# BraveGroup/DCD

Measured on AMD Instinct MI355X. Metric: images/sec DGDE train step (bs=8, 384x1280), higher is better.
Workload: dtype f32; 1 GPU; DGDE train bs=8 fp32 on 1xMI355X, synthetic KITTI 384x1280 + random kpts_ann (DGDE.yaml, DLA-34+DCNv2, 6 objects/image); global_batch=8, per_gpu_batch=8, input=384x1280, parallelism=dp1, dcn_precision=f32, step_launch=eager, sync_bn=False

## Files before the change

### dcd_amd/csrc/conv.hip

```cpp
#include <hip/hip_runtime.h>
#include <stdint.h>
#include <stdlib.h>

#include "../../include/dcd_hip.h"
#include "tuning_env.h"
#include "lds_limit.h"
#include "bf16_split.h"

typedef float f32x16 __attribute__((ext_vector_type(16)));
typedef float f32x4 __attribute__((ext_vector_type(4)));
typedef float f32x2 __attribute__((ext_vector_type(2)));

namespace {

constexpr int WN_CH = 8;
constexpr int WN_NT = 512;

template <int TR, int TC, int NB>
struct WinoGeom {
    static constexpr int KS = 32 * NB;
    static constexpr int U = 16 * KS * WN_CH;
    static constexpr int NTILE = TR * TC;
    static constexpr int ROWS = 4 * TR + 2;
    static constexpr int Q = (2 * TC + 8) / 4;
    static constexpr int RS = TC == 16 ? 48 : 42;
    static constexpr int PLANE = ROWS * RS;
    static constexpr int IN = WN_CH * PLANE;
    static constexpr int BUF = IN + U;
    static_assert(NTILE <= 32 && 4 * Q <= RS && RS % 2 == 0 && (2 * TC) % 4 == 0, "region geometry");
};

__device__ __forceinline__ void win_read4(const float *e, float (&q)[4])
{
    const f32x2 a = *reinterpret_cast<const f32x2 *>(e), b = *reinterpret_cast<const f32x2 *>(e + 2),
                c = *reinterpret_cast<const f32x2 *>(e + 4);
    q[0] = a.y; q[1] = b.x; q[2] = b.y; q[3] = c.x;
}

template <int RS>
__device__ __forceinline__ void win_store4(float *d, const f32x4 v)
{
    if constexpr (RS % 4 == 0) {
        *reinterpret_cast<f32x4 *>(d) = v;
    } else {
        *reinterpret_cast<f32x2 *>(d) = f32x2{v.x, v.y};
        *reinterpret_cast<f32x2 *>(d + 2) = f32x2{v.z, v.w};
    }
}

__device__ __forceinline__ void xcd_remap(int &bx, int &by)
{
    const int gx = gridDim.x, NT = gx * gridDim.y;
    const int L = bx + gx * by;
    const int xc = L & 7, slot = L >> 3;
    const int q = NT >> 3, r = NT & 7;
    const int Lp = (xc < r ? xc * (q + 1) : r * (q + 1) + (xc - r) * q) + slot;
    by = Lp / gx;
    bx = Lp - by * gx;
}

__device__ __forceinline__ void wino_prep_body(const float *__restrict__ w, float *__restrict__ ul, int Cc, int Kk, int mode, int nchunk,
                                               int nz, int WN_KS, int first, int step)
{
    const int n = nz * nchunk * WN_KS * WN_CH;
    for (int idx = first; idx < n; idx += step) {
        int r = idx;
        const int s = r & 3; r >>= 2;
        const int h = r & 1; r >>= 1;
        const int kk = r % WN_KS; r /= WN_KS;
        const int ck = r % nchunk, z = r / nchunk;
        const int k = z * WN_KS + kk, c = ck * WN_CH + 2 * s + h;
        float g[3][3];
#pragma unroll
        for (int a = 0; a < 3; ++a)
#pragma unroll
            for (int b = 0; b < 3; ++b) {
                float v = 0.f;
                if (k < Kk && c < Cc)
                    v = mode == 0 ? w[(((size_t)k * Cc + c) * 3 + a) * 3 + b] : w[(((size_t)c * Kk + k) * 3 + (2 - a)) * 3 + (2 - b)];
                g[a][b] = v;
            }
        float t[4][3];
#pragma unroll
        for (int b = 0; b < 3; ++b) {
            t[0][b] = g[0][b];
            t[1][b] = 0.5f * (g[0][b] + g[1][b] + g[2][b]);
            t[2][b] = 0.5f * (g[0][b] - g[1][b] + g[2][b]);
            t[3][b] = g[2][b];
        }
#pragma unroll
        for (int xi = 0; xi < 4; ++xi) {
            const float u[4] = {t[xi][0], 0.5f * (t[xi][0] + t[xi][1] + t[xi][2]), 0.5f * (t[xi][0] - t[xi][1] + t[xi][2]), t[xi][2]};
#pragma unroll
            for (int nu = 0; nu < 4; ++nu)
                ul[((((size_t)(z * nchunk + ck) * 16 + xi * 4 + nu) * 2 + h) * WN_KS + kk) * 4 + s] = u[nu];
        }
    }
}

__global__ void wino_prep_weights(const float *__restrict__ w, float *__restrict__ ul, int Cc, int Kk, int mode, int nchunk, int nz,
                                  int WN_KS)
{
    wino_prep_body(w, ul, Cc, Kk, mode, nchunk, nz, WN_KS, blockIdx.x * blockDim.x + threadIdx.x, gridDim.x * blockDim.x);
}

struct PrepBoth {
    float *ul[2];
    int Cc[2], Kk[2], nchunk[2], nz[2], ks[2];
};

__global__ void wino_prep_weights_both(const float *__restrict__ w, PrepBoth p)
{
    const int mode = blockIdx.y;
    if (!p.ul[mode]) return;
    wino_prep_body(w, p.ul[mode], p.Cc[mode], p.Kk[mode], mode, p.nchunk[mode], p.nz[mode], p.ks[mode],
                   blockIdx.x * blockDim.x + threadIdx.x, gridDim.x * blockDim.x);
}

__global__ void wino_prep_weights_table(const long long *__restrict__ table)
{
    const long long *e = table + 5 * (size_t)blockIdx.z;
    const float *w = reinterpret_cast<const float *>(e[0]);
    const int mode = blockIdx.y;
    float *ul = reinterpret_cast<float *>(e[1 + mode]);
    if (!w || !ul) return;
    const int Cin = (int)e[3], Cout = (int)e[4];
    const int Cc = mode ? Cout : Cin, Kk = mode ? Cin : Cout;
    const int WN_KS = Kk <= 32 ? 32 : 64;
    wino_prep_body(w, ul, Cc, Kk, mode, (Cc + WN_CH - 1) / WN_CH, (Kk + WN_KS - 1) / WN_KS, WN_KS,
                   blockIdx.x * blockDim.x + threadIdx.x, gridDim.x * blockDim.x);
}

template <int TR, int TC, int NB>
__global__ __launch_bounds__(WN_NT) void wino_conv3x3_f32(const float *__restrict__ x, const float *__restrict__ ul, float *y,
                                                          float *__restrict__ part, const float *__restrict__ bias,
                                                          const float *residual, int Cc, int H, int W, int Kk, int tiles_x,
                                                          int nchunk, int nz)
{
    using G = WinoGeom<TR, TC, NB>;
    constexpr int WN_ROWS = G::ROWS, WN_RS = G::RS, WN_PLANE = G::PLANE, WN_IN = G::IN, WN_BUF = G::BUF, WN_Q = G::Q;
    constexpr int WN_KS = G::KS, WN_U = G::U;
    extern __shared__ __attribute__((aligned(16))) float lds[];
    const int tid = threadIdx.x;
    const int lane = tid & 63, wave = tid >> 6;
    const int p = lane & 31, h = lane >> 5;
    const int xi = wave & 3, tg = wave >> 2;
    int bx = blockIdx.x, b = blockIdx.y;
    xcd_remap(bx, b);
    const int ty = bx / tiles_x, tx = bx - ty * tiles_x;
    const int r0 = ty * (4 * TR), c0 = tx * (2 * TC);
    const int z = blockIdx.z % nz, ks = blockIdx.z / nz, ksplit = gridDim.z / nz;
    const int ck0 = (int)((int64_t)ks * nchunk / ksplit), ck1 = (int)((int64_t)(ks + 1) * nchunk / ksplit);
    const int HW = H * W;
    const bool live = p < G::NTILE;
    const int pe = live ? p : 0;
    const int trow = pe / TC, tcol = pe - trow * TC;

    const int ra = xi == 0 ? 0 : 1, rb = xi == 3 ? 3 : 2;
    const float sa = xi == 2 ? -1.f : 1.f, sb = (xi == 0 || xi == 3) ? -1.f : 1.f;
    const int lanebase = (2 * TR * tg + 2 * trow) * WN_RS + 2 + 2 * tcol + h * WN_PLANE;
    const int base1 = lanebase + ra * WN_RS, base2 = lanebase + rb * WN_RS;

    const float *x_b = x + (size_t)b * Cc * HW;
    const float *ul_z = ul + (size_t)z * nchunk * WN_U;

    constexpr int KIN = (WN_CH * WN_ROWS * WN_Q + WN_NT - 1) / WN_NT;
    constexpr int KW = WN_U / 4 / WN_NT;
    int sg[KIN], sl[KIN];
    bool sv_[KIN];
#pragma unroll
    for (int k = 0; k < KIN; ++k) {
        const int e = tid + WN_NT * k;
        const int ch = e / (WN_ROWS * WN_Q), rem = e - ch * (WN_ROWS * WN_Q);
        const int row = rem / WN_Q, q = rem - row * WN_Q;
        const int yy = r0 - 1 + row, xx = c0 - 4 + 4 * q;
        sv_[k] = e < WN_CH * WN_ROWS * WN_Q;
        sg[k] = (sv_[k] && yy >= 0 && yy < H && xx >= 0 && xx < W) ? ch * HW + yy * W + xx : -1;
        sl[k] = ch * WN_PLANE + row * WN_RS + 4 * q;
    }
    f32x4 rin[KIN];
    auto issue_w = [&](int ck, float *buf) {
        const float *src = ul_z + (size_t)ck * WN_U + 4 * tid;
        float *dst = buf + WN_IN + 4 * 64 * __builtin_amdgcn_readfirstlane(wave);
#pragma unroll
        for (int k = 0; k < KW; ++k)
            __builtin_amdgcn_global_load_lds(src + 4 * WN_NT * k, (__attribute__((address_space(3))) void *)(dst + 4 * WN_NT * k), 16, 0, 0);
    };
    auto issue = [&](int ck) {
        const float *src = x_b + (size_t)ck * WN_CH * HW;
        const int cleft = Cc - ck * WN_CH;
#pragma unroll
        for (int k = 0; k < KIN; ++k) {
            const f32x4 zero4 = {0.f, 0.f, 0.f, 0.f};
            rin[k] = zero4;
            if (sv_[k] && sg[k] >= 0 && (tid + WN_NT * k) / (WN_ROWS * WN_Q) < cleft) rin[k] = *reinterpret_cast<const f32x4 *>(src + sg[k]);
        }
    };
    auto commit = [&](float *buf) {
#pragma unroll
        for (int k = 0; k < KIN; ++k)
            if (sv_[k]) win_store4<WN_RS>(buf + sl[k], rin[k]);
    };

    f32x16 acc[4][NB];
#pragma unroll
    for (int nu = 0; nu < 4; ++nu)
#pragma unroll
        for (int mb = 0; mb < NB; ++mb)
#pragma unroll
            for (int r = 0; r < 16; ++r) acc[nu][mb][r] = 0.f;

    issue_w(ck0, lds);
    issue(ck0);
    commit(lds);
    asm volatile("s_waitcnt vmcnt(0)" ::: "memory");
    __syncthreads();

    for (int ck = ck0; ck < ck1; ++ck) {
        const float *buf = lds + ((ck - ck0) & 1) * WN_BUF;
#ifndef WN_ABL_NOSTAGE
        if (ck + 1 < ck1) {
            issue_w(ck + 1, lds + ((ck + 1 - ck0) & 1) * WN_BUF);
            issue(ck + 1);
        }
#endif
        const float *ub = buf + WN_IN + ((xi * 4 * 2 + h) * WN_KS + p) * 4;
        const float *cp1 = buf + base1, *cp2 = buf + base2;
        f32x4 a0[4], a1[4];
#pragma unroll
        for (int nu = 0; nu < 4; ++nu) {
            a0[nu] = *reinterpret_cast<const f32x4 *>(ub + (nu * WN_KS) * 8);
            if (NB == 2) a1[nu] = *reinterpret_cast<const f32x4 *>(ub + (nu * WN_KS) * 8 + 32 * 4);
        }
        float qa[4], qb[4];
#ifndef WN_ABL_NOLDS
        win_read4(cp1, qa);
        win_read4(cp2, qb);
#endif
#pragma unroll
        for (int s = 0; s < 4; ++s) {
#ifdef WN_ABL_NOLDS
            const float t0 = sa * (float)s, t1 = sb, t2 = sa + sb, t3 = (float)ck;
#else
            const float t0 = sa * qa[0] + sb * qb[0], t1 = sa * qa[1] + sb * qb[1];
            const float t2 = sa * qa[2] + sb * qb[2], t3 = sa * qa[3] + sb * qb[3];
            if (s + 1 < 4) {
                win_read4(cp1 + 2 * (s + 1) * WN_PLANE, qa);
                win_read4(cp2 + 2 * (s + 1) * WN_PLANE, qb);
            }
#endif
            const float v[4] = {t0 - t2, t1 + t2, t2 - t1, t1 - t3};
            __builtin_amdgcn_sched_barrier(0);
#pragma unroll
            for (int nu = 0; nu < 4; ++nu) {
                acc[nu][0] = __builtin_amdgcn_mfma_f32_32x32x2f32(a0[nu][s], v[nu], acc[nu][0], 0, 0, 0);
                if (NB == 2) acc[nu][NB - 1] = __builtin_amdgcn_mfma_f32_32x32x2f32(a1[nu][s], v[nu], acc[nu][NB - 1], 0, 0, 0);
            }
        }
#ifndef WN_ABL_NOSTAGE
        if (ck + 1 < ck1) commit(lds + ((ck + 1 - ck0) & 1) * WN_BUF);
#endif
        asm volatile("s_waitcnt vmcnt(0)" ::: "memory");
        __syncthreads();
    }
#ifdef WN_ABL_NOEPI
    if (acc[0][0][0] != 123.456f) return;
#endif

    float *ex = lds;
    float *y_b = (ks == 0 ? y : part + (size_t)(ks - 1) * gridDim.y * Kk * HW) + (size_t)b * Kk * HW;
    const float *r_b = (residual && ks == 0) ? residual + (size_t)b * Kk * HW : nullptr;
    const int orow0 = r0 + 2 * TR * tg + 2 * trow, ocol = c0 + 2 * tcol;
#pragma unroll
    for (int mb = 0; mb < NB; ++mb) {
        float *mine = ex + (size_t)wave * 32 * 64 + lane;
#pragma unroll
        for (int r = 0; r < 16; ++r) {
            mine[r * 64] = acc[0][mb][r] + acc[1][mb][r] + acc[2][mb][r];
            mine[(16 + r) * 64] = acc[1][mb][r] - acc[2][mb][r] - acc[3][mb][r];
        }
        __syncthreads();
        const float *t0 = ex + (size_t)(tg * 4 + 0) * 32 * 64 + lane, *t1 = t0 + 32 * 64, *t2 = t1 + 32 * 64, *t3 = t2 + 32 * 64;
        if (live && ocol < W) {
#pragma unroll
            for (int rr = 0; rr < 4; ++rr) {
                const int r = 4 * xi + rr;
                const int k = z * WN_KS + mb * 32 + (r & 3) + 8 * (r >> 2) + 4 * h;
                const float a0 = t0[r * 64], a1 = t1[r * 64], a2 = t2[r * 64], a3 = t3[r * 64];
                const float b0 = t0[(16 + r) * 64], b1 = t1[(16 + r) * 64], b2 = t2[(16 + r) * 64], b3 = t3[(16 + r) * 64];
                if (k < Kk) {
                    const float bk = (bias && ks == 0) ? bias[k] : 0.f;
                    const size_t o = (size_t)k * HW + (size_t)orow0 * W + ocol;
                    float *dst = y_b + o;
                    f32x2 r0 = {bk, bk}, r1 = {bk, bk};
                    if (r_b) {
                        if (orow0 < H) r0 += *reinterpret_cast<const f32x2 *>(r_b + o);
                        if (orow0 + 1 < H) r1 += *reinterpret_cast<const f32x2 *>(r_b + o + W);
                    }
                    if (orow0 < H) *reinterpret_cast<f32x2 *>(dst) = f32x2{a0 + a1 + a2 + r0.x, b0 + b1 + b2 + r0.y};
                    if (orow0 + 1 < H) *reinterpret_cast<f32x2 *>(dst + W) = f32x2{a1 - a2 - a3 + r1.x, b1 - b2 - b3 + r1.y};
                }
            }
        }
        __syncthreads();
    }
}

constexpr int WS_CH = 16;

template <int NB>
__device__ __forceinline__ void wino_prep_split_body(const float *__restrict__ w, unsigned *__restrict__ us, int Cc, int Kk, int mode,
                                                     int nchunk, int nz, int first, int step)
{
    constexpr int KS = 32 * NB;
    const int n = nz * nchunk * KS * 2 * 4;
    for (int idx = first; idx < n; idx += step) {
        int r = idx;
        const int d = r & 3; r >>= 2;
        const int h = r & 1; r >>= 1;
        const int kk = r % KS; r /= KS;
        const int ck = r % nchunk, z = r / nchunk;
        const int k = z * KS + kk;
        float u[2][16];
#pragma unroll
        for (int e = 0; e < 2; ++e) {
            const int c = ck * WS_CH + 2 * (2 * d + e) + h;
            float g[3][3];
#pragma unroll
            for (int a = 0; a < 3; ++a)
#pragma unroll
                for (int b = 0; b < 3; ++b) {
                    float v = 0.f;
                    if (k < Kk && c < Cc)
                        v = mode == 0 ? w[(((size_t)k * Cc + c) * 3 + a) * 3 + b] : w[(((size_t)c * Kk + k) * 3 + (2 - a)) * 3 + (2 - b)];
                    g[a][b] = v;
                }
            float t[4][3];
#pragma unroll
            for (int b = 0; b < 3; ++b) {
                t[0][b] = g[0][b];
                t[1][b] = 0.5f * (g[0][b] + g[1][b] + g[2][b]);
                t[2][b] = 0.5f * (g[0][b] - g[1][b] + g[2][b]);
                t[3][b] = g[2][b];
            }
#pragma unroll
            for (int xi = 0; xi < 4; ++xi) {
                u[e][xi * 4 + 0] = t[xi][0];
// ... 500 lines not shown

__global__ __launch_bounds__(256) void wino_wrw_reduce(const float *__restrict__ part, float *__restrict__ gw, int Cin, int Cout, int S,
                                                       int ncg, int KO)
{
    __shared__ float m[12][17];
    const int tid = threadIdx.x;
    const int pos = tid >> 4, l = tid & 15;
    const int gidx = blockIdx.x * 16 + l;
    const int per = KO * 64;
    const int blk = gidx / per, kc = gidx - blk * per;
    if (pos < 12) {
        const float *src = part + ((size_t)blk * S * 12 + pos) * per + kc;
        float sum = 0.f;
#pragma unroll 8
        for (int sp = 0; sp < S; ++sp) sum += src[(size_t)sp * 12 * per];
        m[pos][l] = sum;
    }
    __syncthreads();
    if (pos < 9) {
        const int a = pos / 3, b = pos - a * 3;
        const float ga[4] = {a == 0 ? 1.f : 0.f, 0.5f, a == 1 ? -0.5f : 0.5f, a == 2 ? 1.f : 0.f};
        float r = 0.f;
#pragma unroll
        for (int xi = 0; xi < 4; ++xi) r += ga[xi] * m[xi * 3 + b][l];
        const int og = blk / ncg, cg = blk - og * ncg;
        const int k = og * KO + (kc >> 6), c = cg * 64 + (kc & 63);
        if (k < Cout && c < Cin) gw[((size_t)k * Cin + c) * 9 + pos] = r;
    }
}

}

struct ConvPlan {
    int geom;
    int nb;
    int tiles_x, tiles_y, nchunk, nz, ksplit;
};

static int device_cus()
{
    static int cus = 0;
    if (!cus) {
        int dev = 0, n = 0;
        if (hipGetDevice(&dev) != hipSuccess || hipDeviceGetAttribute(&n, hipDeviceAttributeMultiprocessorCount, dev) != hipSuccess || n <= 0)
            n = 256;
        cus = n;
    }
    return cus;
}

static ConvPlan conv_plan(int B, int Cc, int H, int W, int Kk)
{
    ConvPlan best{};
    const int cus = device_cus();
    int64_t best_cost = -1;
    for (int g = 0; g < 2; ++g) {
        ConvPlan p;
        p.geom = g;
        p.tiles_x = g == 0 ? (W + 31) / 32 : (W + 19) / 20;
        p.tiles_y = g == 0 ? (H + 7) / 8 : (H + 11) / 12;
        p.nchunk = (Cc + WN_CH - 1) / WN_CH;
        p.nb = Kk <= 32 ? 1 : 2;
        p.nz = (Kk + 32 * p.nb - 1) / (32 * p.nb);
        const int64_t wgs = (int64_t)p.tiles_x * p.tiles_y * B * p.nz;
        static const int min_chunks = dcd_env("DCD_CONV_MINCHUNK") ? atoi(dcd_env("DCD_CONV_MINCHUNK")) : 4;
        int ks = 1;
        while (ks < 8 && wgs * (ks * 2) <= cus && p.nchunk / (ks * 2) >= min_chunks) ks *= 2;
        p.ksplit = ks;
        const int64_t rounds = (wgs * ks + cus - 1) / cus;
        const int64_t cost = rounds * ((p.nchunk + ks - 1) / ks + 2) * (g == 0 ? 16 : 17);
        if (best_cost < 0 || cost < best_cost) {
            best_cost = cost;
            best = p;
        }
    }
    return best;
}

template <int TR, int TC, int NB>
static int conv_launch(hipStream_t stream, const ConvPlan &pl, const float *input, const float *ul, float *output, float *part,
                       const float *bias, const float *residual, int B, int Cc, int H, int W, int Kk)
{
    static LdsLimit lds_limit;
    size_t ldsb = (size_t)2 * WinoGeom<TR, TC, NB>::BUF * sizeof(float);
    if (ldsb < (size_t)8 * 32 * 64 * sizeof(float)) ldsb = (size_t)8 * 32 * 64 * sizeof(float);
    if (!lds_limit.raise((int)ldsb, wino_conv3x3_f32<TR, TC, NB>)) return DCD_ERR_LAUNCH;
    hipLaunchKernelGGL((wino_conv3x3_f32<TR, TC, NB>), dim3(pl.tiles_x * pl.tiles_y, B, pl.nz * pl.ksplit), dim3(WN_NT), ldsb, stream,
                       input, ul, output, part, bias, residual, Cc, H, W, Kk, pl.tiles_x, pl.nchunk, pl.nz);
    return DCD_OK;
}

template <int NB, int NP>
static int conv_launch_split(hipStream_t stream, const ConvPlan &pl, const float *input, const unsigned *us, float *output, float *part,
                             const float *bias, const float *residual, int B, int Cc, int H, int W, int Kk)
{
    static LdsLimit lds_limit;
    using G = WinoGeom<2, 16, NB>;
    const size_t ldsb = ((size_t)((WS_CH * G::PLANE + 3) & ~3) + (size_t)2 * 16 * NB * 2 * 256) * sizeof(float);
    if (!lds_limit.raise((int)ldsb, wino_conv3x3_split<NB, NP>)) return DCD_ERR_LAUNCH;
    hipLaunchKernelGGL((wino_conv3x3_split<NB, NP>), dim3(pl.tiles_x * pl.tiles_y, B, pl.nz * pl.ksplit), dim3(WN_NT), ldsb, stream, input,
                       us, output, part, bias, residual, Cc, H, W, Kk, pl.tiles_x, pl.nchunk, pl.nz);
    return DCD_OK;
}

static ConvPlan conv_plan_split(int B, int Cc, int H, int W, int Kk)
{
    ConvPlan p;
    p.geom = 0;
    p.tiles_x = (W + 31) / 32;
    p.tiles_y = (H + 7) / 8;
    p.nchunk = (Cc + WS_CH - 1) / WS_CH;
    p.nb = Kk <= 32 ? 1 : 2;
    p.nz = (Kk + 32 * p.nb - 1) / (32 * p.nb);
    const int64_t wgs = (int64_t)p.tiles_x * p.tiles_y * B * p.nz;
    const int cus = device_cus();
    int ks = 1;
    while (ks < 8 && wgs * (ks * 2) <= cus && p.nchunk / (ks * 2) >= 2) ks *= 2;
    p.ksplit = ks;
    return p;
}

static bool conv_direct_ok(int Cc, int H, int W)
{
    return (int64_t)(Cc + DC_CH) * H * W < (1ll << 29);
}

static ConvPlan conv_plan_direct(int B, int Cc, int H, int W, int Kk)
{
    static const int pin = dcd_env("DCD_CONV_DIRECT_P") ? atoi(dcd_env("DCD_CONV_DIRECT_P")) : 0;
    const int cus = device_cus();
    ConvPlan best{};
    int64_t best_cost = -1;
    for (int P = 2; P <= 4; P += 2) {
        if (P != (pin == 4 ? 4 : 2)) continue;
        ConvPlan p;
        static const int wxpin = dcd_env("DCD_CONV_DIRECT_WX") ? atoi(dcd_env("DCD_CONV_DIRECT_WX")) : 0;
        const int wx = P == 2 && wxpin == 2 ? 2 : 1;
        p.geom = P | (wx << 4);
        p.tiles_x = (W + 32 * wx - 1) / (32 * wx);
        p.tiles_y = (H + 4 * P - 1) / (4 * P);
        p.nchunk = (Cc + DC_CH - 1) / DC_CH;
        p.nb = Kk <= 32 ? 1 : 2;
        p.nz = (Kk + 32 * p.nb - 1) / (32 * p.nb);
        const int64_t wgs = (int64_t)p.tiles_x * p.tiles_y * B * p.nz;
        static const int min_chunks = dcd_env("DCD_CONV_DIRECT_MINCHUNK") ? atoi(dcd_env("DCD_CONV_DIRECT_MINCHUNK")) : 16;
        int ks = 1;
        while (ks < 8) {
            const int64_t next = wgs * ks * 2;
            const int left = p.nchunk / (ks * 2);
            const bool fill = next <= 3 * cus && left >= min_chunks;
            const bool small = 2 * next <= 3 * cus && left >= 2;
            if (!fill && !small) break;
            ks *= 2;
        }
        p.ksplit = ks;
        best = p;
    }
    (void)best_cost;
    return best;
}

template <int NB, int P, int MODE, int WX>
static int conv_launch_direct(hipStream_t stream, const ConvPlan &pl, const float *input, const unsigned *wd, float *output, float *part,
                              const float *bias, const float *residual, int B, int Cc, int H, int W, int Kk)
{
    static LdsLimit lds_limit;
    const size_t ldsb = ((size_t)2 * (4 * P + 2) * (32 * WX + 8) + (size_t)2 * 9 * NB * 64) * 16;
// ... 551 lines not shown
```

### dcd_amd/csrc/dcn_v2.hip

```cpp

#include <hip/hip_runtime.h>
#include <stdint.h>
#include <stdlib.h>
#include <string.h>
#include <atomic>
#include <map>
#include <vector>
#include <mutex>
#include <utility>

#include "../../include/dcd_hip.h"
#include "tuning_env.h"
#include "lds_limit.h"

typedef float f32x16 __attribute__((ext_vector_type(16)));
typedef float f32x32 __attribute__((ext_vector_type(32)));

namespace {

template <int N> struct IntC {
    static constexpr int value = N;
};

struct Geom {
// ... 360 lines not shown
                    vt[u] = ldg2(ipc, to[t0 + u][0]);
                    vb[u] = ldg2(ipc, to[t0 + u][1]);
#pragma unroll
                    for (int mb = 0; mb < MB; ++mb) a[u][mb] = ldg(wpc, wlane + (unsigned)(t0 + u) * Cop4 + mb * 128u);
                }
#pragma unroll
                for (int u = 0; u < 3; ++u) {
                    float val = tw[t0 + u][0] * vt[u].x + tw[t0 + u][1] * vt[u].y + tw[t0 + u][2] * vb[u].x + tw[t0 + u][3] * vb[u].y;
                    val = live ? val : 0.f;
#pragma unroll
                    for (int mb = 0; mb < MB; ++mb)
                        acc[mb] = __builtin_amdgcn_mfma_f32_32x32x2f32(a[u][mb], val, acc[mb], 0, 0, 0);
                }
            }
        };
        for (int it = 0; it < npair; ++it)
            pair_step((const float *)((const char *)ip + (size_t)it * 2 * HW4),
                      (const float *)((const char *)wp + (size_t)it * 18 * Cop4), true);
        if (g.cpg & 1) {
            const size_t back = h ? (size_t)g.H * g.W : 0;
            const size_t wback = h ? (size_t)9 * g.Cop : 0;
            pair_step((const float *)((const char *)ip + (size_t)npair * 2 * HW4) - back,
                      (const float *)((const char *)wp + (size_t)npair * 18 * Cop4) - wback, h == 0);
        }
    }

    float *out_b = out + (size_t)b * g.Co * g.HoWo;
#pragma unroll
    for (int mb = 0; mb < MB; ++mb) {
        const int obase = (ob0 + mb) * 32 + 4 * h;
#pragma unroll
        for (int r = 0; r < 16; ++r) {
            const int o = obase + (r & 3) + 8 * (r >> 2);
            if (pv && o < g.Co) out_b[(size_t)o * g.HoWo + Pc] = acc[mb][r] + bias[o];
        }
    }
}

typedef float f32x4 __attribute__((ext_vector_type(4)));

__global__ void dcn_prep_weights_tile(const float *__restrict__ w, float *__restrict__ wl, Geom g, int nchunk, int nz,
                                      unsigned *__restrict__ flags, int nflag_words, float *__restrict__ wf9)
{
    for (int i = blockIdx.x * blockDim.x + threadIdx.x; i < nflag_words; i += gridDim.x * blockDim.x) flags[i] = 0u;
    if (wf9) {
        const int K = g.C * 9, n9 = K * g.Cop;
        for (int idx = blockIdx.x * blockDim.x + threadIdx.x; idx < n9; idx += gridDim.x * blockDim.x) {
            const int k = idx / g.Cop, o = idx - k * g.Cop;
            wf9[idx] = (o < g.Co) ? w[(size_t)o * K + k] : 0.f;
        }
    }
    const int n = nz * nchunk * TL_W_FLOATS;
    for (int idx = blockIdx.x * blockDim.x + threadIdx.x; idx < n; idx += gridDim.x * blockDim.x) {
        int r = idx;
        const int s = r & 3; r >>= 2;
        const int h = r & 1; r >>= 1;
        const int o = r % TL_OB; r /= TL_OB;
        const int t = r % 9; r /= 9;
        const int ck = r % nchunk, z = r / nchunk;
        const int oo = z * TL_OB + o, c = ck * TL_CH + 2 * s + h;
        wl[idx] = (oo < g.Co && c < g.C) ? w[((size_t)oo * g.C + c) * 9 + t] : 0.f;
    }
}

constexpr float TL_NEAR_F = 3.f;
__global__ __launch_bounds__(256) void dcn_fwd_far_count(const float *__restrict__ off, int64_t n, unsigned *__restrict__ counter)
{
    unsigned c = 0;
    const int64_t n4 = ((uintptr_t)off & 15) == 0 ? n >> 2 : 0;
    for (int64_t i = (int64_t)blockIdx.x * blockDim.x + threadIdx.x; i < n4; i += (int64_t)gridDim.x * blockDim.x) {
        const f32x4 v = *reinterpret_cast<const f32x4 *>(off + 4 * i);
        c += (!(fabsf(v.x) < TL_NEAR_F)) + (!(fabsf(v.y) < TL_NEAR_F)) + (!(fabsf(v.z) < TL_NEAR_F)) + (!(fabsf(v.w) < TL_NEAR_F));
    }
    for (int64_t i = 4 * n4 + (int64_t)blockIdx.x * blockDim.x + threadIdx.x; i < n; i += (int64_t)gridDim.x * blockDim.x)
        c += !(fabsf(off[i]) < TL_NEAR_F);
#pragma unroll
    for (int o = 32; o > 0; o >>= 1) c += __shfl_xor(c, o);
    __shared__ unsigned part[4];
    if ((threadIdx.x & 63) == 0) part[threadIdx.x >> 6] = c;
    __syncthreads();
    if (threadIdx.x == 0 && part[0] + part[1] + part[2] + part[3]) atomicAdd(counter, part[0] + part[1] + part[2] + part[3]);
}

template <int TR>
__global__ __launch_bounds__(TR * 64) void dcn_fwd_tile_f32(const float *__restrict__ in, const float *__restrict__ off,
                                                        const float *__restrict__ msk, const float *__restrict__ wl,
                                                        const float *__restrict__ bias, float *__restrict__ out, Geom g,
                                                        int tiles_x, int nchunk, unsigned char *__restrict__ rescue_flags,
                                                        const float *__restrict__ wf9, int rescue_taps,
                                                        const unsigned *__restrict__ far_count, unsigned far_limit)
{
    typedef TileCfg<TR> T;
    constexpr int TL_ROWS = TR, TL_WH = T::WH, TL_PLANE = T::PLANE, TL_IN_FLOATS = T::IN_FLOATS, TL_BUF = T::BUF,
                  TL_NIN = T::NIN, NT = T::NT, KIN = T::KIN, KW = T::KW;
    extern __shared__ __attribute__((aligned(16))) float lds[];
    const int tid = threadIdx.x;
    const int lane = tid & 63, wave = tid >> 6;
    const int p = lane & 31, h = lane >> 5;
    int bx = blockIdx.x, b = blockIdx.y;
    xcd_remap(bx, b);
    if (*far_count > far_limit) {
        if (tid == 0) rescue_flags[(size_t)b * gridDim.x + bx] = 1;
        return;
    }
    const int ty = bx / tiles_x, tx = bx - ty * tiles_x;
    const int r0 = ty * TL_ROWS, c0 = tx * 32;
    const int ho = r0 + wave, wo = c0 + p;
    const bool pv = ho < g.Ho && wo < g.Wo;
    const int Pc = pv ? ho * g.Wo + wo : 0;
    const int z = blockIdx.z;
    const int HW = g.H * g.W;
    const int Y0 = r0 - 4, X0 = c0 - 4;

    const float *in_b = in + (size_t)b * g.C * HW;
    const float *off_b = off + (size_t)b * 18 * g.HoWo;
    const float *msk_b = msk + (size_t)b * 9 * g.HoWo;
    const float *wl_z = wl + (size_t)z * nchunk * TL_W_FLOATS;

    int sg[KIN], sl[KIN];
    bool sv_[KIN];
#pragma unroll
    for (int k = 0; k < KIN; ++k) {
        const int e = tid + NT * k;
        const int ch = e / (TL_WH * 10), rem = e - ch * (TL_WH * 10);
        const int row = rem / 10, q = rem - row * 10;
        const int y = Y0 + row, x = X0 + 4 * q;
        sv_[k] = e < TL_NIN;
        sg[k] = (sv_[k] && y >= 0 && y < g.H && x >= 0 && x < g.W) ? ch * HW + y * g.W + x : -1;
        sl[k] = ch * TL_PLANE + row * TL_WW + 4 * q;
    }
    f32x4 rin[KIN];
    auto issue_w = [&](int ck, float *buf) {
        const float *src = wl_z + (size_t)ck * TL_W_FLOATS + 4 * tid;
        float *dst = buf + TL_IN_FLOATS + 4 * 64 * __builtin_amdgcn_readfirstlane(wave);
#pragma unroll
        for (int k = 0; k < KW; ++k)
            if (64 * __builtin_amdgcn_readfirstlane(wave) + NT * k < TL_NW)
                __builtin_amdgcn_global_load_lds(src + 4 * NT * k, (__attribute__((address_space(3))) void *)(dst + 4 * NT * k), 16, 0, 0);
    };
    auto issue = [&](int ck) {
        const float *src = in_b + (size_t)ck * TL_CH * HW;
        const int cleft = g.C - ck * TL_CH;
#pragma unroll
        for (int k = 0; k < KIN; ++k) {
            const f32x4 zero4 = {0.f, 0.f, 0.f, 0.f};
            rin[k] = zero4;
            if (sv_[k] && sg[k] >= 0 && (tid + NT * k) / (TL_WH * 10) < cleft) rin[k] = *reinterpret_cast<const f32x4 *>(src + sg[k]);
        }
    };
    auto commit = [&](float *buf) {
#pragma unroll
        for (int k = 0; k < KIN; ++k)
            if (sv_[k]) *reinterpret_cast<f32x4 *>(buf + sl[k]) = rin[k];
    };

    issue(0);

    int lo[9];
    float wq[9][4];
    unsigned farbits = 0;
#pragma unroll
    for (int t = 0; t < 9; ++t) {
        const TapRaw raw = load_tap_raw(off_b, msk_b, g, t, Pc);
        const float hf = (float)(ho - 1 + t / 3) + raw.oh, wf_ = (float)(wo - 1 + t % 3) + raw.ow;
        const bool sv = pv && hf > -1.f && wf_ > -1.f && hf < (float)g.H && wf_ < (float)g.W;
        const float hlf = floorf(hf), wlf = floorf(wf_);
        const int ly = sv ? (int)hlf - Y0 : 0, lx = sv ? (int)wlf - X0 : 0;
        const bool inside = ly >= 0 && lx >= 0 && ly <= TL_WH - 2 && lx <= TL_WW - 2;
        farbits |= (sv && !inside) ? (1u << t) : 0u;
        lo[t] = (inside ? ly * TL_WW + lx : 0) + h * TL_PLANE;
        const float lh = hf - hlf, lw = wf_ - wlf;
        const float m = (sv && inside) ? raw.m : 0.f;
        wq[t][0] = (1.f - lh) * (1.f - lw) * m; wq[t][1] = (1.f - lh) * lw * m;
        wq[t][2] = lh * (1.f - lw) * m;         wq[t][3] = lh * lw * m;
    }

    f32x16 acc[2];
#pragma unroll
    for (int mb = 0; mb < 2; ++mb)
#pragma unroll
        for (int r = 0; r < 16; ++r) acc[mb][r] = 0.f;

    int wave_far_taps = 0;
#pragma unroll
    for (int t = 0; t < 9; ++t) wave_far_taps += __any((farbits >> t) & 1u) ? 1 : 0;
    __shared__ int far_worst;
    if (tid == 0) far_worst = 0;
    __syncthreads();
    if (lane == 0) atomicMax(&far_worst, wave_far_taps);
    __syncthreads();
    if (far_worst >= rescue_taps) {
        if (tid == 0) rescue_flags[(size_t)b * gridDim.x + bx] = 1;
        return;
    }

    issue_w(0, lds);
    commit(lds);
    asm volatile("s_waitcnt vmcnt(0)" ::: "memory");
    __syncthreads();

    for (int ck = 0; ck < nchunk; ++ck) {
        const float *buf = lds + (ck & 1) * TL_BUF;
#ifndef TL_ABL_NOSTAGE
        if (ck + 1 < nchunk) {
            issue_w(ck + 1, lds + ((ck + 1) & 1) * TL_BUF);
            issue(ck + 1);
        }
#endif
        const float *wb_ = buf + TL_IN_FLOATS + (p * 2 + h) * 4;
#pragma unroll
        for (int t = 0; t < 9; ++t) {
#ifdef TL_ABL_NOW
            const f32x4 a0 = {wq[t][0], wq[t][1], wq[t][2], wq[t][3]}, a1 = {wq[t][1], wq[t][0], wq[t][3], wq[t][2]};
            (void)wb_;
#else
            const f32x4 a0 = *reinterpret_cast<const f32x4 *>(wb_ + (t * TL_OB) * 8);
            const f32x4 a1 = *reinterpret_cast<const f32x4 *>(wb_ + (t * TL_OB + 32) * 8);
#endif
            const float *cp = buf + lo[t];
            const float q0 = wq[t][0], q1 = wq[t][1], q2 = wq[t][2], q3 = wq[t][3];
#pragma unroll
            for (int s = 0; s < 4; ++s) {
                const float *c2 = cp + 2 * s * TL_PLANE;
#ifdef TL_ABL_NOLDS
                const float val = q0 * (float)s + q1 + q2 * (float)ck + q3;
                (void)c2;
#else
                const float val = q0 * c2[0] + q1 * c2[1] + q2 * c2[TL_WW] + q3 * c2[TL_WW + 1];
#endif
                acc[0] = __builtin_amdgcn_mfma_f32_32x32x2f32(a0[s], val, acc[0], 0, 0, 0);
                acc[1] = __builtin_amdgcn_mfma_f32_32x32x2f32(a1[s], val, acc[1], 0, 0, 0);
            }
        }
#ifndef TL_ABL_NOSTAGE
        if (ck + 1 < nchunk) commit(lds + ((ck + 1) & 1) * TL_BUF);
#endif
        asm volatile("s_waitcnt vmcnt(0)" ::: "memory");
#ifndef TL_ABL_NOBAR
        __syncthreads();
#endif
    }

    if (__any(farbits != 0u)) {
#pragma unroll 1
        for (int t = 0; t < 9; ++t) {
            if (!__any((farbits >> t) & 1u)) continue;
            const bool mine = (farbits >> t) & 1u;
            const Tap s = make_tap(off_b, msk_b, g, t, t, ho, wo, Pc, pv);
            const float *w9 = wf9 + (size_t)t * g.Cop + z * TL_OB + p;
            const bool second = z * TL_OB + 32 < g.Cop;
            const int cend = (g.C + 1) & ~1;
            for (int c0 = h; c0 < cend; c0 += 8) {
                f32x2 gt[4], gb[4];
                float wa[4], wb2[4];
#pragma unroll
                for (int u = 0; u < 4; ++u) {
                    const int c = c0 + 2 * u;
                    const int cc = c < g.C ? c : g.C - 1;
                    const float *gp = in_b + (size_t)cc * HW;
                    gt[u] = ldg2(gp, (unsigned)s.pt * 4u);
                    gb[u] = ldg2(gp, (unsigned)s.pb * 4u);
                    const float *wr = w9 + (size_t)cc * 9 * g.Cop;
                    wa[u] = wr[0];
                    wb2[u] = second ? wr[32] : 0.f;
                }
#pragma unroll
                for (int u = 0; u < 4; ++u) {
                    const int c = c0 + 2 * u;
                    const bool live = mine && c < g.C;
                    const float val = live ? (s.a0 * gt[u].x + s.a1 * gt[u].y + s.b0 * gb[u].x + s.b1 * gb[u].y) * s.m : 0.f;
                    acc[0] = __builtin_amdgcn_mfma_f32_32x32x2f32(wa[u], val, acc[0], 0, 0, 0);
                    acc[1] = __builtin_amdgcn_mfma_f32_32x32x2f32(wb2[u], val, acc[1], 0, 0, 0);
                }
            }
        }
    }

    float *out_b = out + (size_t)b * g.Co * g.HoWo;
#pragma unroll
    for (int mb = 0; mb < 2; ++mb) {
        const int obase = z * TL_OB + mb * 32 + 4 * h;
#pragma unroll
        for (int r = 0; r < 16; ++r) {
            const int o = obase + (r & 3) + 8 * (r >> 2);
            if (pv && o < g.Co) out_b[(size_t)o * g.HoWo + ho * g.Wo + wo] = acc[mb][r] + bias[o];
        }
    }
}

constexpr float TL_NEAR = 3.f;
constexpr unsigned FAR_BY_COUNT = 0x80000000u;
constexpr unsigned FAR_COUNT_PIVOT = 0x40000000u;
__device__ __forceinline__ bool far_dominated(const unsigned *far_scal, int total_tiles)
{
    if (!far_scal) return false;
    const unsigned c = far_scal[3];
    if (c & FAR_BY_COUNT) return (c & ~FAR_BY_COUNT) > FAR_COUNT_PIVOT;
    return (int64_t)far_scal[1] * 2 > (int64_t)total_tiles;
}

inline unsigned far_count_limit(const Geom &g, bool wide)
{
    static const int div = dcd_env("DCD_FAR_DIV") ? atoi(dcd_env("DCD_FAR_DIV")) : 0;
    static const int div_wide = dcd_env("DCD_FAR_DIV_WIDE") ? atoi(dcd_env("DCD_FAR_DIV_WIDE")) : 0;
    int d = wide ? div_wide : div;
    if (d <= 0) d = wide ? (g.B >= 4 ? 16 : 8) : (g.B >= 4 ? 24 : 12);
    const int64_t total = (int64_t)g.B * 18 * g.HoWo;
    int64_t lim = total / d;
    if (lim > (int64_t)FAR_COUNT_PIVOT - 1) lim = FAR_COUNT_PIVOT - 1;
    return (unsigned)lim;
}

struct HandoverState {
    unsigned *host = nullptr;
    unsigned *dev = nullptr;
// ... 2070 lines not shown
```

Baseline: 214.3 images/s.

## Software-pipeline LDS reads in Winograd conv and DCN tile kernels

In the Winograd 3x3 conv kernel, the weight slabs move into a triple-buffered LDS ring that is fetched two chunks ahead. The next chunk's A-operand registers are read mid-loop so the LDS reads overlap the MFMAs, and the chunk loop is unrolled by two to ping-pong register sets. In the DCN forward tile kernel, the 36-step tap loop is flattened and uses hand-issued ds_read2/ds_read_b128 instructions with a prefetch ring and explicit lgkmcnt waits, so corner and weight loads overlap MFMA work. This raises LDS footprint and register pressure, and the hand-counted waitcnt values are fragile.

```diff
diff --git a/dcd_amd/csrc/conv.hip b/dcd_amd/csrc/conv.hip
--- a/dcd_amd/csrc/conv.hip
+++ b/dcd_amd/csrc/conv.hip
@@ -26,7 +26,6 @@
     static constexpr int RS = TC == 16 ? 48 : 42;
     static constexpr int PLANE = ROWS * RS;
     static constexpr int IN = WN_CH * PLANE;
-    static constexpr int BUF = IN + U;
     static_assert(NTILE <= 32 && 4 * Q <= RS && RS % 2 == 0 && (2 * TC) % 4 == 0, "region geometry");
 };
 
@@ -35,6 +34,21 @@
     const f32x2 a = *reinterpret_cast<const f32x2 *>(e), b = *reinterpret_cast<const f32x2 *>(e + 2),
                 c = *reinterpret_cast<const f32x2 *>(e + 4);
     q[0] = a.y; q[1] = b.x; q[2] = b.y; q[3] = c.x;
+}
+
+struct WinRow {
+    f32x2 a, b, c;
+};
+__device__ __forceinline__ void win_read_row(const float *e, WinRow &r)
+{
+    r.a = *reinterpret_cast<const f32x2 *>(e);
+    r.b = *reinterpret_cast<const f32x2 *>(e + 2);
+    r.c = *reinterpret_cast<const f32x2 *>(e + 4);
+}
+__device__ __forceinline__ void win_row_vals(const WinRow &r, float (&q)[4])
+{
+    asm volatile("" ::"v"(r.a), "v"(r.c));
+    q[0] = r.a.y; q[1] = r.b.x; q[2] = r.b.y; q[3] = r.c.x;
 }
 
 template <int RS>
@@ -138,7 +152,7 @@
                                                           int nchunk, int nz)
 {
     using G = WinoGeom<TR, TC, NB>;
-    constexpr int WN_ROWS = G::ROWS, WN_RS = G::RS, WN_PLANE = G::PLANE, WN_IN = G::IN, WN_BUF = G::BUF, WN_Q = G::Q;
+    constexpr int WN_ROWS = G::ROWS, WN_RS = G::RS, WN_PLANE = G::PLANE, WN_IN = G::IN, WN_Q = G::Q;
     constexpr int WN_KS = G::KS, WN_U = G::U;
     extern __shared__ __attribute__((aligned(16))) float lds[];
     const int tid = threadIdx.x;
@@ -179,9 +193,9 @@
         sl[k] = ch * WN_PLANE + row * WN_RS + 4 * q;
     }
     f32x4 rin[KIN];
-    auto issue_w = [&](int ck, float *buf) {
+    auto issue_w = [&](int ck, float *slab) {
         const float *src = ul_z + (size_t)ck * WN_U + 4 * tid;
-        float *dst = buf + WN_IN + 4 * 64 * __builtin_amdgcn_readfirstlane(wave);
+        float *dst = slab + 4 * 64 * __builtin_amdgcn_readfirstlane(wave);
 #pragma unroll
         for (int k = 0; k < KW; ++k)
             __builtin_amdgcn_global_load_lds(src + 4 * WN_NT * k, (__attribute__((address_space(3))) void *)(dst + 4 * WN_NT * k), 16, 0, 0);
@@ -210,59 +224,78 @@
 #pragma unroll
             for (int r = 0; r < 16; ++r) acc[nu][mb][r] = 0.f;
 
-    issue_w(ck0, lds);
+    auto read_a = [&](const float *slab, f32x4 (&a0)[4], f32x4 (&a1)[4]) {
+        const float *ub = slab + ((xi * 4 * 2 + h) * WN_KS + p) * 4;
+#pragma unroll
+        for (int nu = 0; nu < 4; ++nu) {
+            a0[nu] = *reinterpret_cast<const f32x4 *>(ub + (nu * WN_KS) * 8);
+            if (NB == 2) a1[nu] = *reinterpret_cast<const f32x4 *>(ub + (nu * WN_KS) * 8 + 32 * 4);
+        }
+    };
+
+    float *const slabs = lds + 2 * WN_IN;
+    issue_w(ck0, slabs);
+    if (ck0 + 1 < ck1) issue_w(ck0 + 1, slabs + WN_U);
     issue(ck0);
     commit(lds);
     asm volatile("s_waitcnt vmcnt(0)" ::: "memory");
     __syncthreads();
 
-    for (int ck = ck0; ck < ck1; ++ck) {
-        const float *buf = lds + ((ck - ck0) & 1) * WN_BUF;
+    f32x4 ra0[2][4], ra1[2][4];
+    read_a(slabs, ra0[0], ra1[0]);
+    int sn1 = 1, sn2 = 2;
+
+    auto chunk = [&](int ck, const f32x4 (&a0)[4], const f32x4 (&a1)[4], f32x4 (&n0)[4], f32x4 (&n1)[4]) {
+        const float *buf = lds + ((ck - ck0) & 1) * WN_IN;
 #ifndef WN_ABL_NOSTAGE
-        if (ck + 1 < ck1) {
-            issue_w(ck + 1, lds + ((ck + 1 - ck0) & 1) * WN_BUF);
-            issue(ck + 1);
-        }
+        if (ck + 2 < ck1) issue_w(ck + 2, slabs + sn2 * WN_U);
+        if (ck + 1 < ck1) issue(ck + 1);
 #endif
-        const float *ub = buf + WN_IN + ((xi * 4 * 2 + h) * WN_KS + p) * 4;
         const float *cp1 = buf + base1, *cp2 = buf + base2;
-        f32x4 a0[4], a1[4];
-#pragma unroll
-        for (int nu = 0; nu < 4; ++nu) {
-            a0[nu] = *reinterpret_cast<const f32x4 *>(ub + (nu * WN_KS) * 8);
-            if (NB == 2) a1[nu] = *reinterpret_cast<const f32x4 *>(ub + (nu * WN_KS) * 8 + 32 * 4);
-        }
-        float qa[4], qb[4];
+        WinRow wa, wb;
 #ifndef WN_ABL_NOLDS
-        win_read4(cp1, qa);
-        win_read4(cp2, qb);
+        win_read_row(cp1, wa);
+        win_read_row(cp2, wb);
 #endif
 #pragma unroll
         for (int s = 0; s < 4; ++s) {
 #ifdef WN_ABL_NOLDS
             const float t0 = sa * (float)s, t1 = sb, t2 = sa + sb, t3 = (float)ck;
 #else
+            float qa[4], qb[4];
+            win_row_vals(wa, qa);
+            win_row_vals(wb, qb);
             const float t0 = sa * qa[0] + sb * qb[0], t1 = sa * qa[1] + sb * qb[1];
             const float t2 = sa * qa[2] + sb * qb[2], t3 = sa * qa[3] + sb * qb[3];
             if (s + 1 < 4) {
-                win_read4(cp1 + 2 * (s + 1) * WN_PLANE, qa);
-                win_read4(cp2 + 2 * (s + 1) * WN_PLANE, qb);
+                win_read_row(cp1 + 2 * (s + 1) * WN_PLANE, wa);
+                win_read_row(cp2 + 2 * (s + 1) * WN_PLANE, wb);
             }
 #endif
             const float v[4] = {t0 - t2, t1 + t2, t2 - t1, t1 - t3};
+            if (s == 1 && ck + 1 < ck1) read_a(slabs + sn1 * WN_U, n0, n1);
             __builtin_amdgcn_sched_barrier(0);
 #pragma unroll
             for (int nu = 0; nu < 4; ++nu) {
                 acc[nu][0] = __builtin_amdgcn_mfma_f32_32x32x2f32(a0[nu][s], v[nu], acc[nu][0], 0, 0, 0);
                 if (NB == 2) acc[nu][NB - 1] = __builtin_amdgcn_mfma_f32_32x32x2f32(a1[nu][s], v[nu], acc[nu][NB - 1], 0, 0, 0);
             }
+            if (s <= 1) __builtin_amdgcn_sched_barrier(0);
         }
 #ifndef WN_ABL_NOSTAGE
-        if (ck + 1 < ck1) commit(lds + ((ck + 1 - ck0) & 1) * WN_BUF);
+        if (ck + 1 < ck1) commit(lds + ((ck + 1 - ck0) & 1) * WN_IN);
 #endif
         asm volatile("s_waitcnt vmcnt(0)" ::: "memory");
         __syncthreads();
-    }
+        sn1 = sn2;
+        sn2 = sn2 == 2 ? 0 : sn2 + 1;
+    };
+    int ck = ck0;
+    for (; ck + 1 < ck1; ck += 2) {
+        chunk(ck, ra0[0], ra1[0], ra0[1], ra1[1]);
+        chunk(ck + 1, ra0[1], ra1[1], ra0[0], ra1[0]);
+    }
+    if (ck < ck1) chunk(ck, ra0[0], ra1[0], ra0[1], ra1[1]);
 #ifdef WN_ABL_NOEPI
     if (acc[0][0][0] != 123.456f) return;
 #endif
@@ -929,7 +962,9 @@
                        const float *bias, const float *residual, int B, int Cc, int H, int W, int Kk)
 {
     static LdsLimit lds_limit;
-    size_t ldsb = (size_t)2 * WinoGeom<TR, TC, NB>::BUF * sizeof(float);
+    using G = WinoGeom<TR, TC, NB>;
+    static_assert(G::IN % 4 == 0 && G::U % 4 == 0, "windows and slabs start on 16 bytes");
+    size_t ldsb = ((size_t)2 * G::IN + (size_t)3 * G::U) * sizeof(float);
     if (ldsb < (size_t)8 * 32 * 64 * sizeof(float)) ldsb = (size_t)8 * 32 * 64 * sizeof(float);
     if (!lds_limit.raise((int)ldsb, wino_conv3x3_f32<TR, TC, NB>)) return DCD_ERR_LAUNCH;
     hipLaunchKernelGGL((wino_conv3x3_f32<TR, TC, NB>), dim3(pl.tiles_x * pl.tiles_y, B, pl.nz * pl.ksplit), dim3(WN_NT), ldsb, stream,
diff --git a/dcd_amd/csrc/dcn_v2.hip b/dcd_amd/csrc/dcn_v2.hip
--- a/dcd_amd/csrc/dcn_v2.hip
+++ b/dcd_amd/csrc/dcn_v2.hip
@@ -466,6 +466,23 @@
     if (threadIdx.x == 0 && part[0] + part[1] + part[2] + part[3]) atomicAdd(counter, part[0] + part[1] + part[2] + part[3]);
 }
 
+__device__ __forceinline__ unsigned lds_addr(const float *p)
+{
+    return (unsigned)(uintptr_t)(const __attribute__((address_space(3))) float *)p;
+}
+
+#define DCD_LGKM_CASE(N) \
+    case N: asm volatile("s_waitcnt lgkmcnt(" #N ")" : "+v"(top), "+v"(bot), "+v"(a0), "+v"(a1)); break;
+__device__ __forceinline__ void lds_wait(int n, f32x2 &top, f32x2 &bot, f32x4 &a0, f32x4 &a1)
+{
+    switch (n) {
+        DCD_LGKM_CASE(1) DCD_LGKM_CASE(2) DCD_LGKM_CASE(3) DCD_LGKM_CASE(4) DCD_LGKM_CASE(5) DCD_LGKM_CASE(6) DCD_LGKM_CASE(7)
+        DCD_LGKM_CASE(8)
+        default: asm volatile("s_waitcnt lgkmcnt(0)" : "+v"(top), "+v"(bot), "+v"(a0), "+v"(a1)); break;
+    }
+}
+#undef DCD_LGKM_CASE
+
 template <int TR>
 __global__ __launch_bounds__(TR * 64) void dcn_fwd_tile_f32(const float *__restrict__ in, const float *__restrict__ off,
                                                         const float *__restrict__ msk, const float *__restrict__ wl,
@@ -592,29 +609,54 @@
         }
 #endif
         const float *wb_ = buf + TL_IN_FLOATS + (p * 2 + h) * 4;
-#pragma unroll
-        for (int t = 0; t < 9; ++t) {
+        constexpr int TL_AHEAD = 2, TL_RING = TL_AHEAD + 1;
+        f32x2 ct[TL_RING], cb[TL_RING];
+        f32x4 wa0[2], wa1[2];
+        auto corners = [&](int i, f32x2 &top, f32x2 &bot) {
+#ifdef TL_ABL_NOLDS
+            top = f32x2{(float)(i & 3), 1.f}; bot = f32x2{(float)ck, 1.f};
+#else
+            const unsigned a = lds_addr(buf + lo[i >> 2] + 2 * (i & 3) * TL_PLANE);
+            asm volatile("ds_read2_b32 %0, %1 offset1:1" : "=v"(top) : "v"(a));
+            asm volatile("ds_read2_b32 %0, %1 offset0:%2 offset1:%3" : "=v"(bot) : "v"(a), "n"(TL_WW), "n"(TL_WW + 1));
+#endif
+        };
+        auto weights = [&](int t, f32x4 &a0, f32x4 &a1) {
 #ifdef TL_ABL_NOW
-            const f32x4 a0 = {wq[t][0], wq[t][1], wq[t][2], wq[t][3]}, a1 = {wq[t][1], wq[t][0], wq[t][3], wq[t][2]};
+            a0 = f32x4{wq[t][0], wq[t][1], wq[t][2], wq[t][3]};
+            a1 = f32x4{wq[t][1], wq[t][0], wq[t][3], wq[t][2]};
             (void)wb_;
 #else
-            const f32x4 a0 = *reinterpret_cast<const f32x4 *>(wb_ + (t * TL_OB) * 8);
-            const f32x4 a1 = *reinterpret_cast<const f32x4 *>(wb_ + (t * TL_OB + 32) * 8);
-#endif
-            const float *cp = buf + lo[t];
-            const float q0 = wq[t][0], q1 = wq[t][1], q2 = wq[t][2], q3 = wq[t][3];
-#pragma unroll
-            for (int s = 0; s < 4; ++s) {
-                const float *c2 = cp + 2 * s * TL_PLANE;
-#ifdef TL_ABL_NOLDS
-                const float val = q0 * (float)s + q1 + q2 * (float)ck + q3;
-                (void)c2;
+            const unsigned a = lds_addr(wb_ + (t * TL_OB) * 8);
+            asm volatile("ds_read_b128 %0, %1" : "=v"(a0) : "v"(a));
+            asm volatile("ds_read_b128 %0, %1 offset:%2" : "=v"(a1) : "v"(a), "n"(32 * 8 * 4));
+#endif
+        };
+        auto younger = [](int i) {
+#if defined(TL_ABL_NOLDS) || defined(TL_ABL_NOW)
+            return 0;
 #else
-                const float val = q0 * c2[0] + q1 * c2[1] + q2 * c2[TL_WW] + q3 * c2[TL_WW + 1];
-#endif
-                acc[0] = __builtin_amdgcn_mfma_f32_32x32x2f32(a0[s], val, acc[0], 0, 0, 0);
-                acc[1] = __builtin_amdgcn_mfma_f32_32x32x2f32(a1[s], val, acc[1], 0, 0, 0);
-            }
+            int n = 2 * (35 - i < TL_AHEAD ? 35 - i : TL_AHEAD);
+            for (int j = i > TL_AHEAD ? i - TL_AHEAD : 0; j <= i; ++j)
+                if ((j & 3) == 0 && (j >> 2) + 1 < 9) n += 2;
+            return n;
+#endif
+        };
+        weights(0, wa0[0], wa1[0]);
+#pragma unroll
+        for (int i = 0; i < TL_AHEAD; ++i) corners(i, ct[i], cb[i]);
+#pragma unroll
+        for (int i = 0; i < 36; ++i) {
+            const int t = i >> 2, s = i & 3;
+            if (i + TL_AHEAD < 36) corners(i + TL_AHEAD, ct[(i + TL_AHEAD) % TL_RING], cb[(i + TL_AHEAD) % TL_RING]);
+            if (s == 0 && t + 1 < 9) weights(t + 1, wa0[(t + 1) & 1], wa1[(t + 1) & 1]);
+            f32x2 &top = ct[i % TL_RING], &bot = cb[i % TL_RING];
+            lds_wait(younger(i), top, bot, wa0[t & 1], wa1[t & 1]);
+            __builtin_amdgcn_sched_barrier(0);
+            const float val = fmaf(wq[t][3], bot.y, fmaf(wq[t][2], bot.x, fmaf(wq[t][0], top.x, wq[t][1] * top.y)));
+            __builtin_amdgcn_sched_barrier(0);
+            acc[0] = __builtin_amdgcn_mfma_f32_32x32x2f32(wa0[t & 1][s], val, acc[0], 0, 0, 0);
+            acc[1] = __builtin_amdgcn_mfma_f32_32x32x2f32(wa1[t & 1][s], val, acc[1], 0, 0, 0);
         }
 #ifndef TL_ABL_NOSTAGE
         if (ck + 1 < nchunk) commit(lds + ((ck + 1) & 1) * TL_BUF);
```

Result: no change. 218.5 images/s (median of 3 runs) (+1.9%).
